# Aqasch/TensorRL-QAS

Measured on AMD Instinct MI355X. Metric: VQE env-steps/sec, higher is better.
Workload: dtype f64

## Files before the change

tensorrl-qas_amd/csrc/ham_layout.h:

```cpp
#pragma once
#include "vqe_geo.h"

#include <algorithm>
#include <cmath>
#include <cstddef>
#include <map>
#include <string>
#include <type_traits>
#include <vector>

namespace vqe {

struct HamHost {
  std::vector<uint32_t> gx_all;
  std::vector<std::vector<int>> group_terms;
  std::vector<uint64_t> hx, hz;
  std::vector<double> hcr, hci;
  bool group_has_im(int g) const {
    for (int k : group_terms[g]) if (hci[k] != 0.0) return true;
    return false;
  }
};

inline bool ham_from_paulis(int n, int n_terms, const uint64_t* xmask, const uint64_t* zmask, const double* coeff, HamHost& H) {
// ... 228 lines not shown
inline SwzChoice choose_bank_swizzle(int lt, const std::vector<uint32_t>& urec, const std::vector<uint32_t>& addr) {
  const size_t NT = (size_t)1 << lt, nu = urec.size();
  std::vector<uint8_t> lo, hi;
  size_t n_scored = 0;
  for (size_t u = 0; u < nu; ++u) {
    if (!urec[u]) continue;
    ++n_scored;
    for (size_t t = 0; t < NT; ++t) {
      const uint32_t p = addr[((u / kUnitTrip) * NT + t) * kUnitTrip + u % kUnitTrip] >> 4;
      lo.push_back((uint8_t)(p & 15u));
      hi.push_back((uint8_t)((p >> 4) & 15u));
    }
  }
  uint8_t grp[4][16];
  for (int g = 0, cnt[4] = {0, 0, 0, 0}; g < 64; ++g) {
    const int k = ((g >> 5) << 1) | (((g >> 2) ^ (g >> 3) ^ (g >> 4)) & 1);
    grp[k][cnt[k]++] = (uint8_t)g;
  }
  auto table = [](const uint32_t (&c)[4]) {
    uint64_t t = 0;
    for (uint32_t v = 0; v < 16; ++v) {
      uint32_t code = 0;
      for (int k = 0; k < 4; ++k) if ((v >> k) & 1u) code ^= c[k];
      t |= (uint64_t)code << (4 * v);
    }
    return t;
  };
  auto score = [&](uint64_t swz, double* worst) {
    size_t tot = 0;
    int w = 1;
    for (size_t i = 0; i < n_scored * NT; i += 64)
      for (int k = 0; k < 4; ++k) {
        int seen[16] = {0}, m = 0;
        for (int l = 0; l < 16; ++l) {
          const size_t j = i + grp[k][l];
          const int s = lo[j] ^ (int)((swz >> (4 * hi[j])) & 15u);
          m = std::max(m, ++seen[s]);
        }
        tot += m;
        w = std::max(w, m);
      }
    if (worst) *worst = w;
    return n_scored ? (double)tot / (double)(n_scored * NT / 16) : 1.0;
  };
  SwzChoice r{0, 1.0, 1.0, 1.0, 1.0};
  if (!n_scored || lt < 8) return r;
  r.mean0 = r.mean = score(0, &r.worst0);
  r.worst = r.worst0;
  const uint32_t starts[2][4] = {{0u, 0u, 0u, 0u}, {1u, 15u, 2u, 12u}};
  for (const auto& st : starts) {
    uint32_t c[4] = {st[0], st[1], st[2], st[3]};
    double best = score(table(c), nullptr);
    for (int sweep = 0; sweep < 4; ++sweep) {
      bool moved = false;
      for (int k = 0; k < 4; ++k)
        for (uint32_t v = 0; v < 16; ++v) {
          const uint32_t keep = c[k];
          c[k] = v;
          const double s = score(table(c), nullptr);
          if (s < best) { best = s; moved = true; } else c[k] = keep;
        }
      if (!moved) break;
    }
    if (best < r.mean) { r.mean = best; r.swz = table(c); }
  }
  if (r.swz) score(r.swz, &r.worst);
  return r;
}

struct HamLayout {
  std::vector<uint32_t> gx;
  std::vector<int32_t> tab_r, tab_i;
  std::vector<double> tables;
  int has_diag = 0;
  int n_real = 0;
  IndexMap im;
  int n_cls = 0;
  uint32_t mrow[16] = {0};
  uint64_t swz = 0;
  double mean0 = 1.0, worst0 = 1.0, mean = 1.0, worst = 1.0;
  std::vector<uint32_t> urec, uaddr;
  std::vector<double> utab;
  std::vector<int32_t> term_off{0};
  std::vector<uint32_t> term_z;
  std::vector<double> term_cr, term_ci;
};

namespace layout_detail {

constexpr const char* kTooLarge = "Hamiltonian too large for the LDS-resident path";

inline bool classify_sparse_groups(const HamHost& H, int n, int unit_F, const std::vector<int>& mine,
                                   std::vector<char>& sparse, std::vector<uint32_t>& dense_xs, std::vector<int>& hole_freq) {
  const IndexMap id = identity_map(n);
  bool any_sparse = false;
  std::vector<double> D;
  std::vector<uint32_t> act;
  std::vector<int> fixed;
  for (int g : mine) {
    const uint32_t x = H.gx_all[g];
    if (!x || H.group_has_im(g)) continue;
    const int sel = top_bit(x);
    double scale;
    pair_table(H, g, id, n, sel, D, &scale, act);
    const int patterns = choose_fixed_bits(n, sel, unit_F, act, fixed);
    const int units = patterns << (unit_F - (int)fixed.size());
    if (2 * units <= (1 << unit_F)) {
      sparse[g] = 1;
      any_sparse = true;
      for (int b : fixed) ++hole_freq[b];
      ++hole_freq[sel];
    } else {
      dense_xs.push_back(x);
    }
  }
  return any_sparse;
}

inline bool build_units(const HamHost& H, int n, int lt, const std::vector<int>& mine, const std::vector<char>& sparse,
                        HamLayout& L, std::string& err) {
  const int unit_F = n - 1 - lt;
  const size_t NT = (size_t)1 << lt;
  std::vector<double> D;
  std::vector<uint32_t> act;
  std::vector<int> fixed;
  for (int g : mine) {
    if (!sparse[g]) continue;
    const uint32_t x = L.im.map_x(H.gx_all[g]);
    const int sel = top_bit(x);
    double scale;
    pair_table(H, g, L.im, n, sel, D, &scale, act);
    choose_fixed_bits(n, sel, unit_F, act, fixed);
    for (int b = n - 1; b >= 0 && (int)fixed.size() < unit_F; --b)
      if (b != sel && std::find(fixed.begin(), fixed.end(), b) == fixed.end()) fixed.push_back(b);
    uint32_t fmask = 0;
    for (int b : fixed) fmask |= 1u << b;
    std::vector<uint32_t> keys;
    for (uint32_t p0 : act) keys.push_back(p0 & fmask);
    std::sort(keys.begin(), keys.end());
    keys.erase(std::unique(keys.begin(), keys.end()), keys.end());
    for (uint32_t s : keys) {
      L.urec.push_back(x << 4);
      for (size_t t = 0; t < NT; ++t) {
        uint32_t p0 = s, tb = 0;
        for (int b = 0; b < n; ++b)
          if (!((fmask >> b) & 1u) && b != sel) { p0 |= (uint32_t)((t >> tb) & 1u) << b; ++tb; }
        const size_t q = ((size_t)(p0 >> (sel + 1)) << sel) | (p0 & (((size_t)1 << sel) - 1));
        const double d = D[q];
        L.utab.push_back(std::fabs(d) > kUnitZeroTol * scale ? d : 0.0);
        L.uaddr.push_back(p0 << 4);
      }
    }
  }
  if (L.utab.size() * sizeof(double) + (size_t)kUnitUnroll * NT * sizeof(double) > 0x7FFFFFFFu) { err = kTooLarge; return false; }
  while (L.urec.size() % kUnitUnroll) {
    L.urec.push_back(0u);
    L.utab.resize(L.utab.size() + NT, 0.0);
    L.uaddr.resize(L.uaddr.size() + NT, 0u);
  }
  auto by_trip = [&](auto& v) {
    std::remove_reference_t<decltype(v)> t(v.size());
    const size_t n_trips = L.urec.size() / kUnitTrip;
    for (size_t T = 0; T < n_trips; ++T)
      for (size_t j = 0; j < (size_t)kUnitTrip; ++j)
        for (size_t th = 0; th < NT; ++th)
          t[(T * NT + th) * kUnitTrip + j] = v[(T * kUnitTrip + j) * NT + th];
    v.swap(t);
  };
  by_trip(L.utab);
  by_trip(L.uaddr);
  return true;
}

inline bool build_group_list(const HamHost& H, int n, bool lds_path, bool reg_path, int lt, std::vector<int> mine,
                             const std::vector<char>& sparse, HamLayout& L, std::string& err) {
  const size_t dim = (size_t)1 << n;
  const IndexMap& im = L.im;
  auto gxm = [&](int g) { return im.map_x(H.gx_all[g]); };
  auto rank_of = [&](int g) {
    if (H.group_has_im(g)) return 3;
    const uint32_t x = gxm(g);
    if (x == 0) return 0;
    return reg_path && (x >> lt) ? 1 : 2;
  };
  if (lds_path)
    std::stable_sort(mine.begin(), mine.end(), [&](int a, int b) {
      return rank_of(a) != rank_of(b) ? rank_of(a) < rank_of(b) : top_bit(gxm(a)) > top_bit(gxm(b));
    });
  auto add_dummy = [&](uint32_t xd) {
    L.gx.push_back(xd);
    L.term_off.push_back((int32_t)L.term_z.size());
    L.tab_r.push_back((int32_t)L.tables.size());
    L.tab_i.push_back(-1);
    L.tables.resize(L.tables.size() + dim / 2, 0.0);
  };
  int cur_rank = 0;
  auto enter_section = [&](int rank) {
    if (lds_path) {
      if (cur_rank <= 1 && rank >= 2) while (L.n_cls % energy_pd(n)) { add_dummy(1u << lt); ++L.n_cls; ++L.n_real; }
      if (cur_rank <= 2 && rank >= 3) while ((L.n_real - L.n_cls) % energy_pd(n)) { add_dummy(1u); ++L.n_real; }
    }
    cur_rank = rank;
  };
  std::vector<uint32_t> pidx;
  for (int g : mine) {
    if (sparse[g]) continue;
    const uint32_t x = gxm(g);
    const bool has_im = H.group_has_im(g);
    const int rank = rank_of(g);
    enter_section(rank);
    L.gx.push_back(x);
    for (int k : H.group_terms[g]) {
      L.term_z.push_back(im.map_z((uint32_t)H.hz[k]));
      L.term_cr.push_back(H.hcr[k]);
      L.term_ci.push_back(H.hci[k]);
    }
    L.term_off.push_back((int32_t)L.term_z.size());
    if (!lds_path) {
      L.tab_r.push_back(0);
      L.tab_i.push_back(has_im ? 0 : -1);
      continue;
    }
    if (rank == 0) L.has_diag = 1; else if (!has_im) ++L.n_real;
    if (rank == 1) ++L.n_cls;
    const size_t len = x == 0 ? dim : dim / 2;
    if (L.tables.size() + 2 * len > 0x7FFFFFFFu) { err = kTooLarge; return false; }
    L.tab_r.push_back((int32_t)L.tables.size());
    L.tables.resize(L.tables.size() + len, 0.0);
    if (has_im) { L.tab_i.push_back((int32_t)L.tables.size()); L.tables.resize(L.tables.size() + len, 0.0); }
    else L.tab_i.push_back(-1);
    double* tr = L.tables.data() + L.tab_r.back();
    double* ti = has_im ? L.tables.data() + L.tab_i.back() : nullptr;
    pidx.resize(len);
    for (size_t q = 0; q < len; ++q) {
      if (x == 0) pidx[q] = (uint32_t)q;
      else if (rank == 1) {
        const uint32_t t = (uint32_t)((q >> 1) & (((size_t)1 << lt) - 1));
        const uint32_t j = (uint32_t)(((q >> (lt + 1)) << 1) | (q & 1));
        pidx[q] = t | (insert0(j, top_bit(x) - lt) << lt);
      } else {
        pidx[q] = insert0((uint32_t)q, top_bit(x));
      }
    }
    for (int k : H.group_terms[g]) {
      const uint32_t z = im.map_z((uint32_t)H.hz[k]);
      const double factor = x == 0 ? 1.0 : 2.0;
      add_sign_term(tr, 1, pidx, z, factor, H.hcr[k]);
      if (ti) add_sign_term(ti, 1, pidx, z, factor, H.hci[k]);
    }
  }
  enter_section(4);
  return true;
}

}

inline bool plan_hamiltonian(const HamHost& H, int n, bool lds_path, int rank, int world, bool units_on, HamLayout& L,
                             std::string& err) {
  using namespace layout_detail;
  L = HamLayout{};
  const std::vector<int> mine = shard_groups(H, lds_path, rank, world);
  const bool reg_path = lds_path && n >= kRegMinQubits;
  const int lt = geo_lt(n);
  const int unit_F = n - 1 - lt;
  L.im = identity_map(n);
  std::vector<char> sparse(H.gx_all.size(), 0);
  bool any_sparse = false;
  if (lds_path && n >= kUnitMinQubits && units_on && unit_F >= 1) {
    std::vector<int> hole_freq(n, 0);
    std::vector<uint32_t> dense_xs;
    any_sparse = classify_sparse_groups(H, n, unit_F, mine, sparse, dense_xs, hole_freq);
    if (any_sparse && reg_path)
      L.im = choose_permutation(n, lt, dense_xs, hole_freq);
  }
  if (reg_path && !any_sparse) {
    std::vector<uint32_t> xs;
    for (int g : mine) if (H.gx_all[g] && !H.group_has_im(g)) xs.push_back(H.gx_all[g]);
    L.im = choose_index_map(n, lt, xs);
  }
  if (any_sparse && !build_units(H, n, lt, mine, sparse, L, err)) return false;
  if (!build_group_list(H, n, lds_path, reg_path, lt, mine, sparse, L, err)) return false;
  if (reg_path && !L.urec.empty() && L.gx.size() == (size_t)(L.has_diag + L.n_cls)) {
    const SwzChoice sw = choose_bank_swizzle(lt, L.urec, L.uaddr);
    L.swz = sw.swz; L.mean0 = sw.mean0; L.worst0 = sw.worst0; L.mean = sw.mean; L.worst = sw.worst;
  }
  if (L.swz) {
    for (uint32_t& a : L.uaddr) a = swz_slot(L.swz, a >> 4) << 4;
    for (uint32_t& x : L.urec) x = swz_slot(L.swz, x >> 4) << 4;
  }
  for (int i = 0; i < 16; ++i) {
    uint32_t row = L.im.row[i];
    for (int k = 0; i < 4 && k < 4; ++k)
      if ((L.swz >> (4 * (1 << k)) >> i) & 1u) row ^= L.im.row[4 + k];
    L.mrow[i] = row;
  }
  return true;
}

struct GradTables {
  std::vector<uint32_t> gx;
  std::vector<int64_t> off;
  std::vector<int32_t> cplx;
  std::vector<double> tab;
};

inline void plan_grad_tables(const HamHost& H, int n, bool lds_path, int rank, int world, GradTables& T) {
  T = GradTables{};
  const size_t dim = (size_t)1 << n;
  std::vector<uint32_t> rep;
  for (int g : shard_groups(H, lds_path, rank, world)) {
    const uint32_t x = H.gx_all[g];
    const bool im = H.group_has_im(g);
    rep.resize(x == 0 ? dim : dim / 2);
    for (size_t q = 0; q < rep.size(); ++q) rep[q] = x == 0 ? (uint32_t)q : insert0((uint32_t)q, top_bit(x));
    T.gx.push_back(x);
    T.off.push_back((int64_t)T.tab.size());
    T.cplx.push_back(im ? 1 : 0);
    const size_t base = T.tab.size();
    T.tab.resize(base + (im ? 2 : 1) * rep.size(), 0.0);
    double* t = T.tab.data() + base;
    for (int k : H.group_terms[g]) {
      add_sign_term(t, im ? 2 : 1, rep, (uint32_t)H.hz[k], 1.0, H.hcr[k]);
      if (im) add_sign_term(t + 1, 2, rep, (uint32_t)H.hz[k], 1.0, H.hci[k]);
    }
  }
}

}
```

tensorrl-qas_amd/csrc/vqe_api.hip:

```cpp
#include "../../include/vqe_hip.h"
#include "vqe_device.h"
#include "vqe_devbuf.h"
#include "vqe_stream.h"
#include "vqe_dm.h"
#include "vqe_dm_batch.h"
#include "vqe_dm_grad.h"
#include "vqe_grad.h"
#include "vqe_lbfgs.h"
#include "vqe_stream_lbfgs.h"
#include "vqe_lanczos.h"
#include "vqe_qjump.h"
#include "vqe_stream_qjump.h"
#include "ham_layout.h"
#include "dm_host.h"
#include "env_step_host.h"

#include <algorithm>
#include <cassert>
#include <cmath>
#include <cstdio>
#include <cstdlib>
#include <cstring>
#include <dlfcn.h>
#include <map>
// ... 30 lines not shown
  hipStream_t own_stream = nullptr, stream = nullptr;
  hipEvent_t ev0 = nullptr, ev1 = nullptr;
  float last_ms = 0.f;
  std::string err;

  DevBuf<double2> init;
  HamHost ham_host;
  int shard_rank = 0, shard_world = 1;
  int amp_rank = 0, amp_world = 1;
  bool ham_set = false;
  DevBuf<uint32_t> d_gx, d_term_z;
  DevBuf<double> d_term_cr, d_term_ci, d_tables;
  DevBuf<int32_t> d_tab_r, d_tab_i;

  DevBuf<int32_t> d_term_off;
  DevBuf<uint32_t> d_urec;
  DevBuf<uint32_t> d_uaddr;
  DevBuf<double> d_utab;
  HamDev ham{};
  double unit_score[4] = {1.0, 1.0, 1.0, 1.0};
  NoiseCfg noise{0.0, 0.0, 0ull, 0ull, 0.0};
  double pauli_w1[3] = {}, pauli_w2[15] = {};
  NoisePauliTab pauli_tab{};
  DevBuf<NoisePauliTab> d_pauli_tab;

  std::vector<GateRec> circ;
  int circ_params = -1;

  int batch = 0;
  int64_t total_params = 0;
  int max_ops = 0, max_params = 0, max_pair = 0;
  std::vector<int64_t> h_par_begin;
  std::vector<int32_t> h_par_count;
  DevBuf<GateRec> d_gates;
  DevBuf<int64_t> d_gate_begin, d_par_begin, d_scratch_begin;
  DevBuf<int32_t> d_gate_count, d_par_count, d_nfev, d_new_gate, d_order;
  bool has_new_gate = false;
  std::vector<int32_t> h_gate_count;
  std::vector<GateRec> h_gates;
  std::vector<int64_t> h_gate_begin;
  std::vector<double> h_theta;
  std::vector<int32_t> h_new_gate;
  DevBuf<GateRec> d_gates2;
  DevBuf<int64_t> d_gate_begin2, d_par_begin2;
  DevBuf<int32_t> d_gate_count2, d_par_count2;
  DevBuf<double> d_theta, d_x, d_xraw, d_f, d_scratch;
  DevBuf<double2> d_state;
  DevBuf<unsigned long long> d_dbg;
  DevBuf<double> d_trace;
  bool trace_on = false;
  int trace_maxfun = 0, trace_stride = 0, trace_batch = 0;
  int noise_mode = 0;
  DevBuf<double2> dm_rho;
  DevBuf<double> dm_S, dm_partial, dm_cr, dm_ci;
  DevBuf<uint32_t> dm_gx, dm_tz;
  DevBuf<int32_t> dm_toff;
  int dm_groups = 0, dm_blocks_last = 0;
  float dm_gpu_ms = 0.f;
  bool last_run_dm = false;
  hipEvent_t dm_ev0 = nullptr, dm_ev1 = nullptr;
  uint64_t dm_ham_gen = ~0ull;
  int dm_batched = 0;
  size_t dm_auto_cap = 0;
  int64_t dm_info[4] = {0, 0, 0, 0};
  DevBufExact<double2> dmb_rho;
  DevBuf<double> dmb_partial;
  DmPlanSlot dmb_full, dmb_pre;
  bool dm_grad = false;
  DmKraus kraus;
  DmKraus channels;
  bool dm_rot2 = false;
  DevBuf<double> dmg_part;
  DevBuf<int32_t> dmg_active;
  DevBuf<double> ls_xres, ls_fres;
  DevBuf<int32_t> ls_nfres, ls_running;
  DevBuf<double> d_cob_x0;
  DevBuf<int32_t> d_cob_active;
  void* comm = nullptr;
  int comm_world = 0;
  StreamWork sw;
  uint64_t gen = 0;
  uint64_t ham_ver = 0, grad_ham_ver = ~0ull;
  DevBuf<uint32_t> g_gx;
  DevBuf<int64_t> g_off;
  DevBuf<int32_t> g_cplx;
  DevBuf<double> g_tab, d_grad;
  DevBuf<double2> g_lam;
  GradHam gham{};
  DevBuf<double> lb_work;
  DevBuf<int32_t> lb_nit, lb_status;
  int lb_batch = 0;
  bool stream_grad = false, stream_states_undone = false;
  bool stream_lbfgs = false;
  DevBufExact<StreamLbfgsRec> lb_rec;
  int kraus_traj = 0;
  uint64_t qj_ver = 0, qj_tab_ver = ~0ull;
  DevBuf<double> qj_K1, qj_W1, qj_K2, qj_W2, qj_e;
  DevBuf<int32_t> qj_jumps;
  DevBuf<long long> qj_jsum;
  int qj_n1 = 0, qj_n2 = 0;
  int64_t qj_info[4] = {0, 0, 0, 0};
  int qj_traj_batch = 0;
  int qj_jsum_batch = 0;
  int sq_resident = 0;
  size_t sq_auto_cap = 0;
  int64_t sq_info[4] = {0, 0, 0, 0};
  DevBuf<QjOp> sq_ops;
  DevBuf<uint32_t> sq_masks;
  DevBuf<int32_t> sq_meta, sq_jpos;
  DevBuf<double2> sq_cs;
  DevBuf<double> sq_part, sq_kmat;
  LzWork lz;
};

#ifdef VQE_STAMPS
static unsigned long long cby_out_[8];
#endif
namespace {

int fail(vqe_t* h, int code, const std::string& msg) {
  if (h) h->err = msg; else g_create_error = msg;
  return code;
}

template <class T>
int upload(vqe_t* h, DevBuf<T>& b, const T* src, size_t n) {
  HIP_TRY(h, b.reserve(n ? n : 1));
  if (n) HIP_TRY(h, hipMemcpyAsync(b.p, src, n * sizeof(T), hipMemcpyHostToDevice, h->stream));
  return VQE_OK;
}
template <class T>
int upload(vqe_t* h, DevBuf<T>& b, const std::vector<T>& src) { return upload(h, b, src.data(), src.size()); }

int build_hamiltonian(vqe_t* h, HamHost* H, int rank, int world) {
  static const bool units_on = [] { const char* e = std::getenv("VQE_UNITS"); return !(e && e[0] == '0'); }();
  HamLayout L;
  std::string err;
  if (!plan_hamiltonian(H ? *H : h->ham_host, h->n, h->lds_path, rank, world, units_on, L, err))
    return fail(h, VQE_EINVAL, err);
  if (H) h->ham_host = std::move(*H);
  h->shard_rank = rank;
  h->shard_world = world;
  h->ham_set = true;
  ++h->gen;
  ++h->ham_ver;
  VQE_TRY(upload(h, h->d_gx, L.gx));
  VQE_TRY(upload(h, h->d_tab_r, L.tab_r));
  VQE_TRY(upload(h, h->d_tab_i, L.tab_i));
  VQE_TRY(upload(h, h->d_tables, L.tables));
  VQE_TRY(upload(h, h->d_term_off, L.term_off));
  VQE_TRY(upload(h, h->d_term_z, L.term_z));
  VQE_TRY(upload(h, h->d_term_cr, L.term_cr));
  VQE_TRY(upload(h, h->d_term_ci, L.term_ci));
  VQE_TRY(upload(h, h->d_urec, L.urec));
  VQE_TRY(upload(h, h->d_uaddr, L.uaddr));
  VQE_TRY(upload(h, h->d_utab, L.utab));
  HIP_TRY(h, hipStreamSynchronize(h->stream));
  HamDev& d = h->ham;
  d.n_groups = (int)L.gx.size();
  d.n_terms = (int)L.term_z.size();
  d.n_units = (int)L.urec.size();
  d.gx = h->d_gx.p; d.tab_r = h->d_tab_r.p; d.tab_i = h->d_tab_i.p; d.tables = h->d_tables.p;
  d.urec = h->d_urec.p; d.uaddr = h->d_uaddr.p; d.utab = h->d_utab.p;
  d.term_off = h->d_term_off.p; d.term_z = h->d_term_z.p; d.term_cr = h->d_term_cr.p; d.term_ci = h->d_term_ci.p;
  d.has_diag = L.has_diag; d.n_real = L.n_real; d.n_cls = L.n_cls;
  std::copy(L.mrow, L.mrow + 16, d.mrow);
  d.swz = L.swz;
  h->unit_score[0] = L.mean0; h->unit_score[1] = L.worst0; h->unit_score[2] = L.mean; h->unit_score[3] = L.worst;
  return VQE_OK;
}

int check_gates(vqe_t* h, int64_t n_gates, const int32_t* kind, const int32_t* q0,
                const int32_t* q1, const int32_t* pidx, int n_params) {
  for (int64_t i = 0; i < n_gates; ++i) {
    const int k = kind[i];
    if (k < 0 || k > VQE_GATE_RZZ) return fail(h, VQE_EINVAL, "unknown gate kind");
    if (q0[i] < 0 || q0[i] >= h->n) return fail(h, VQE_EINVAL, "gate qubit out of range");
    if (k == VQE_GATE_CNOT || k == VQE_GATE_DEPOL2 || gate_is_rot2(k)) {
      if (q1[i] < 0 || q1[i] >= h->n || q1[i] == q0[i])
        return fail(h, VQE_EINVAL, "two-qubit gate needs two distinct qubits in range");
    }
    if (gate_is_rot(k)) {
      if (pidx[i] < 0 || pidx[i] >= n_params)
        return fail(h, VQE_EINVAL, "rotation parameter index out of range");
    }
  }
  return VQE_OK;
}

enum class Run { Energy, Minimize, State, EnvStep, Reduce };

void set_env_step(const vqe_t* h, BatchArgs& A) {
  A.env_step = 1;
  A.new_gate = h->has_new_gate ? h->d_new_gate.p : nullptr;
}

#ifdef VQE_ONLY_N
using LdsSizes = std::integer_sequence<int, VQE_ONLY_N>;
#else
using LdsSizes = std::integer_sequence<int, 1, 2, 3, 4, 5, 6, 7, 8, 9, 10, 11, 12, 13>;
#endif
template <class F, int... Ns>
int dispatch_n(vqe_t* h, const char* refusal, F f, std::integer_sequence<int, Ns...>) {
  int rc = 0;
  const bool found = (... || (h->n == Ns && ((rc = f(std::integral_constant<int, Ns>{})), true)));
  return found ? rc : fail(h, VQE_EINVAL, refusal);
}

constexpr int kWideMinN = 6;
bool wide_launch(int n, int max_params) {
  static const bool wide_on = [] { const char* e = std::getenv("VQE_WIDE_UPDATE"); return !(e && e[0] == '0'); }();
  return n >= kWideMinN && wide_on && max_params > 64;
}

const char* lds_launch_refusal(int n, size_t lds, int max_ops, size_t lds_per_cu) {
  if (lds > lds_per_cu) return "circuit too large for the LDS-resident path (gates + parameters)";
  if (n >= kRegMinQubits && (size_t)max_ops > ((size_t)1 << n))
    return "circuit too large for the LDS-resident path (more than 2^n rotations)";
  return nullptr;
}

void report_placement(int n, int max_ops, int max_pair, int max_params, int n_groups, int nvar, bool wide, size_t lds_per_cu,
                      int64_t out[8]) {
  const bool resident = cobyla_resident_bytes(n, max_ops, max_params, n_groups, max_pair) != 0;
  const CobPlacement p = cobyla_placement(n, wide, resident, nvar);
  const size_t lds = lds_bytes(n, max_ops, max_params, n_groups, max_pair, wide);
  out[0] = p.resident ? VQE_COBYLA_RESIDENT : p.staged ? VQE_COBYLA_STAGED : p.block ? VQE_COBYLA_BLOCK
           : p.rows ? VQE_COBYLA_ROWS : VQE_COBYLA_GLOBAL;
  out[1] = p.pad;
  out[2] = p.words;
  out[3] = (int64_t)lds;
  out[4] = p.split;
  out[5] = (int64_t)cobyla_tile_bytes(n, max_params, wide);
  out[6] = (int64_t)cobyla_resident_bytes(n, max_ops, max_params, n_groups, max_pair);
  out[7] = lds_launch_refusal(n, lds, max_ops, lds_per_cu) == nullptr;
}

template <int N>
int launch_lds(vqe_t* h, Run mode, BatchArgs A) {
  if (mode == Run::EnvStep) set_env_step(h, A);
  const bool minimize = mode == Run::Minimize || mode == Run::EnvStep;
  constexpr bool kHasWide = N >= kWideMinN;
  const bool wide = minimize && wide_launch(N, A.max_params);
  size_t lds = lds_bytes(N, A.max_ops, A.max_params, A.ham.n_groups, A.max_pair, wide);
  static const long lds_pad = [] { const char* e = std::getenv("VQE_LDS_PAD"); return e ? std::atol(e) : 0L; }();
  if (lds_pad > 0) lds += (size_t)lds_pad;
  if (const char* why = lds_launch_refusal(N, lds, A.max_ops, (size_t)h->lds_per_cu)) return fail(h, VQE_EINVAL, why);
  const bool noisy = A.noise.p1 > 0.0 || A.noise.p2 > 0.0;
  constexpr bool kW = false;
  void (*const kernel)(BatchArgs) =
      mode == Run::Energy ? k_lds_energy<N>
      : !minimize ? k_lds_state<N>
      : wide ? (noisy ? k_lds_minimize<N, kHasWide, true> : k_lds_minimize<N, kHasWide, false>)
             : (noisy ? k_lds_minimize<N, kW, true> : k_lds_minimize<N, kW, false>);
  const void* fn = (const void*)kernel;
  HIP_TRY(h, hipFuncSetAttribute(fn, hipFuncAttributeMaxDynamicSharedMemorySize, (int)lds));
  {
    hipFuncAttributes fa;
    HIP_TRY(h, hipFuncGetAttributes(&fa, fn));
    if (fa.sharedSizeBytes != 0) return fail(h, VQE_ESTATE, "LDS-resident kernel was built with static LDS");
  }
  h->last_wg_per_cu = std::max(1, std::min(8, (int)(h->lds_per_cu / lds)));
  HIP_TRY(h, hipEventRecord(h->ev0, h->stream));
  const dim3 grid(mode == Run::State ? 1 : A.batch), block(Geo<N>::NT);
  hipLaunchKernelGGL(kernel, grid, block, lds, h->stream, A);
  HIP_TRY(h, hipGetLastError());
  HIP_TRY(h, hipEventRecord(h->ev1, h->stream));
  return VQE_OK;
}

int dispatch_lds(vqe_t* h, Run mode, const BatchArgs& A) {
  return dispatch_n(h, "n_qubits outside the LDS-resident range",
                    [&](auto n) -> int { return launch_lds<decltype(n)::value>(h, mode, A); }, LdsSizes{});
}

NoiseCfg launch_noise(const vqe_t* h) {
  NoiseCfg nz = h->noise;
  if (h->pauli_tab.has1) nz.p1 = h->pauli_tab.cum1[2];
  if (h->pauli_tab.has2) nz.p2 = h->pauli_tab.cum2[14];
  nz.pauli = (h->pauli_tab.has1 || h->pauli_tab.has2) ? h->d_pauli_tab.p : nullptr;
  return nz;
}
bool pauli_noise_on(const vqe_t* h) {
  const NoiseCfg nz = launch_noise(h);
  return nz.p1 > 0.0 || nz.p2 > 0.0;
}
void set_channels(vqe_t* h) {
  h->channels = h->kraus;
  if (h->kraus.n1 == 0 && h->pauli_tab.has1) { pauli_kraus(h->pauli_w1, 2, h->channels.K1); h->channels.n1 = 4; }
  if (h->kraus.n2 == 0 && h->pauli_tab.has2) { pauli_kraus(h->pauli_w2, 4, h->channels.K2); h->channels.n2 = 16; }
}

BatchArgs make_args(vqe_t* h) {
  BatchArgs A{};
  A.n = h->n;
  A.batch = h->batch;
  A.gates = h->d_gates.p;
  A.gate_begin = h->d_gate_begin.p;
  A.gate_count = h->d_gate_count.p;
  A.par_begin = h->d_par_begin.p;
  A.par_count = h->d_par_count.p;
  A.order = h->d_order.p;
  A.theta = h->d_theta.p;
  A.xout = h->d_x.p;
  A.xraw = h->d_xraw.p;
  A.new_gate = nullptr;
  A.env_step = 0;
  A.fout = h->d_f.p;
  A.nfev = h->d_nfev.p;
  A.scratch = h->d_scratch.p;
  A.scratch_begin = h->d_scratch_begin.p;
  A.init = h->init.p;
  A.ham = h->ham;
  A.noise = launch_noise(h);
// ... 2121 lines not shown
```

tensorrl-qas_amd/csrc/vqe_device.h:

```cpp
#pragma once
#include <hip/hip_runtime.h>
#include <stdint.h>
#ifdef VQE_STAMPS
__device__ unsigned long long g_cby_dbg[8];
__device__ unsigned long long g_cby_in_out[2];
__device__ long long g_cby_t0_unused;
#if defined(__HIP_DEVICE_COMPILE__)
#define CBY_STAMP_RESET() long long cby_t0_ = (long long)__builtin_readcyclecounter(); (void)cby_t0_
#define CBY_STAMP(k)                                                                               \
  {                                                                                                \
    const long long t_ = (long long)__builtin_readcyclecounter();                                  \
    if (ctx.tid == 0 && Ctx::nth > 1) __hip_atomic_fetch_add(&g_cby_dbg[k], (unsigned long long)(t_ - cby_t0_), __ATOMIC_RELAXED, __HIP_MEMORY_SCOPE_AGENT); \
    cby_t0_ = (long long)__builtin_readcyclecounter();                                             \
  }
#else
#define CBY_STAMP_RESET()
#define CBY_STAMP(k)
#endif
#endif
#include "cobyla_m0.h"
#include "vqe_geo.h"
#include "noise_pauli.h"

namespace vqe {
// ... 873 lines not shown
      const double* treal = tables + __builtin_amdgcn_readfirstlane(L.gm[g0].off_r);
      VQE_E_CTX(VQE_E_XFETCH(g0))
      xq = VQE_E_XFETCH(g0 + 1);
      VQE_E_LOAD(0, aA, bA)
      for (int g = g0; g < g1; g += PD) {
#pragma unroll
        for (int j = 0; j < PD; ++j) {
          {
            const int sl = (j + PD - 1) % PD;
            int gr = (j == 0) ? (g == g0 ? g0 + PD - 1 : g - 1 + PD) : g + j - 1 + PD;
            gr = gr < g1 ? gr : g1 - 1;
            const double* t = treal + (size_t)(gr - g0) * (DIM / 2);
#pragma unroll
            for (int k = 0; k < NP; ++k) buf[sl][k] = t[tid + (uint32_t)k * kThreads];
          }
          VQE_E_LOAD(1, aB, bB)
          __builtin_amdgcn_sched_barrier(0);
          VQE_E_COMP(0, aA, bA, buf[j])
          __builtin_amdgcn_sched_barrier(0);
          VQE_E_CTX(xq)
          xq = VQE_E_XFETCH(g + j + 2);
          VQE_E_LOAD(0, aA, bA)
          __builtin_amdgcn_sched_barrier(0);
          VQE_E_COMP(1, aB, bB, buf[j])
          __builtin_amdgcn_sched_barrier(0);
        }
      }
#undef VQE_E_CTX
#undef VQE_E_XFETCH
#undef VQE_E_LOAD
#undef VQE_E_COMP
    } else {
      for (int g = g0; g < g1; g += PD) {
        const int gn = g + PD < g1 ? g + PD : g;
#pragma unroll
        for (int j = 0; j < PD; ++j) {
          VQE_ENERGY_CONSUME(g + j, buf[j])
          const double* t = tables + __builtin_amdgcn_readfirstlane(L.gm[gn + j].off_r);
#pragma unroll
          for (int k = 0; k < NP; ++k) {
            const uint32_t q = tid + (uint32_t)k * kThreads;
            buf[j][k] = (FULL || q < DIM / 2) ? t[q] : 0.0;
          }
          __builtin_amdgcn_sched_barrier(0);
        }
      }
    }
  }
}

template <int N>
__device__ __forceinline__ void energy_imag_lds(const Lds& L, const double* __restrict__ tables, int g1, int g2,
                                                double& acc0) {
  constexpr int kThreads = Geo<N>::NT;
  constexpr uint32_t DIM = 1u << N;
  constexpr int NP = (DIM / 2 + kThreads - 1) / kThreads;
  constexpr bool FULL = DIM / 2 >= kThreads;
  const uint32_t tid = threadIdx.x;
  for (int g = g1; g < g2; ++g) {
    const GroupMeta m = L.gm[g];
    const double* tr = tables + m.off_r;
    const double* ti = tables + m.off_i;
    double part = 0.0;
#pragma unroll
    for (int k = 0; k < NP; ++k) {
      const uint32_t q = tid + (uint32_t)k * kThreads;
      if (FULL || q < DIM / 2) {
        const uint32_t p0 = insert0(q, m.hb);
        const double2 b = L.psi[p0], a = L.psi[p0 ^ m.x];
        part += (a.x * b.x + a.y * b.y) * tr[q] - (a.x * b.y - a.y * b.x) * ti[q];
      }
    }
    acc0 += part;
  }
}

template <int N>
__device__ __forceinline__ void unit_energy(const Lds& L, const HamDev& H, double& acc0, double& acc1);

template <int N>
__device__ __forceinline__ double lds_energy(const Lds& L, const HamDev& H) {
  constexpr int kThreads = Geo<N>::NT;
  constexpr uint32_t DIM = 1u << N;
  constexpr int NA = (DIM + kThreads - 1) / kThreads;
  const uint32_t tid = threadIdx.x;
  const double* __restrict__ tables = H.tables;
  double acc0 = 0.0, acc1 = 0.0;
  int g0 = 0;
  if (H.has_diag) {
    const double* t = tables + L.gm[0].off_r;
#pragma unroll
    for (int k = 0; k < NA; ++k) {
      const uint32_t p = tid + (uint32_t)k * kThreads;
      if (DIM >= kThreads || p < DIM) {
        const double2 a = L.psi[p];
        const double v = (a.x * a.x + a.y * a.y) * t[p];
        if (k & 1) acc1 += v; else acc0 += v;
      }
    }
    g0 = 1;
  }
  const int g1 = g0 + H.n_real;
  energy_real_lds<N>(L, tables, g0, g1, acc0, acc1);
  energy_imag_lds<N>(L, tables, g1, H.n_groups, acc0);
  if constexpr (N >= kUnitMinQubits && N - 1 - Geo<N>::LT >= 1) unit_energy<N>(L, H, acc0, acc1);
  return block_sum<Geo<N>::NW>(acc0 + acc1, L.red);
}


__device__ __forceinline__ __amdgpu_buffer_rsrc_t table_rsrc(const void* p) {
  return __builtin_amdgcn_make_buffer_rsrc((void*)p, 0, -1, 0x00020000);
}
__device__ __forceinline__ double2 buf_load_d2(__amdgpu_buffer_rsrc_t rs, uint32_t voff, uint32_t soff) {
  const v4i_t v = __builtin_amdgcn_raw_buffer_load_b128(rs, (int)voff, (int)soff, 0);
  return make_double2(__hiloint2double(v.y, v.x), __hiloint2double(v.w, v.z));
}
__device__ __forceinline__ double buf_load_d(__amdgpu_buffer_rsrc_t rs, uint32_t voff, uint32_t soff) {
  const v2i_t v = __builtin_amdgcn_raw_buffer_load_b64(rs, (int)voff, (int)soff, 0);
  return __hiloint2double(v.y, v.x);
}
__device__ __forceinline__ double2 lds_load_d2(lds_cbyte* base, uint32_t off) {
  const d2v_t v = *(const __attribute__((address_space(3))) d2v_t*)(base + off);
  return make_double2(v.x, v.y);
}

__device__ __forceinline__ void pair_fma4(double& acc0, double& acc1, const double2& a0, const double2& a1,
                                          const double2& a2, const double2& a3, const double2 (&b)[4], double d0,
                                          double d1, double d2, double d3) {
  double t0, t1, t2, t3;
  asm("v_mul_f64 %2, %6, %14\n\tv_mul_f64 %3, %8, %16\n\tv_mul_f64 %4, %10, %18\n\tv_mul_f64 %5, %12, %20\n\t"
      "v_fmac_f64 %2, %7, %15\n\tv_fmac_f64 %3, %9, %17\n\tv_fmac_f64 %4, %11, %19\n\tv_fmac_f64 %5, %13, %21\n\t"
      "v_fmac_f64 %0, %2, %22\n\tv_fmac_f64 %1, %3, %23\n\tv_fmac_f64 %0, %4, %24\n\tv_fmac_f64 %1, %5, %25"
      : "+v"(acc0), "+v"(acc1), "=&v"(t0), "=&v"(t1), "=&v"(t2), "=&v"(t3)
      : "v"(a0.x), "v"(a0.y), "v"(a1.x), "v"(a1.y), "v"(a2.x), "v"(a2.y), "v"(a3.x), "v"(a3.y),
        "v"(b[0].x), "v"(b[0].y), "v"(b[1].x), "v"(b[1].y), "v"(b[2].x), "v"(b[2].y), "v"(b[3].x), "v"(b[3].y),
        "v"(d0), "v"(d1), "v"(d2), "v"(d3));
}
__device__ __forceinline__ void pair_fma2(double& acc0, double& acc1, const double2& a0, const double2& a1,
                                          const double2 (&b)[2], double d0, double d1) {
  double t0, t1;
  asm("v_mul_f64 %2, %4, %8\n\tv_mul_f64 %3, %6, %10\n\t"
      "v_fmac_f64 %2, %5, %9\n\tv_fmac_f64 %3, %7, %11\n\t"
      "v_fmac_f64 %0, %2, %12\n\tv_fmac_f64 %1, %3, %13"
      : "+v"(acc0), "+v"(acc1), "=&v"(t0), "=&v"(t1)
      : "v"(a0.x), "v"(a0.y), "v"(a1.x), "v"(a1.y), "v"(b[0].x), "v"(b[0].y), "v"(b[1].x), "v"(b[1].y),
        "v"(d0), "v"(d1));
}
__device__ __forceinline__ void pair_fma1(double& acc0, const double2& a0, const double2 (&b)[1], double d0) {
  double t0;
  asm("v_mul_f64 %1, %2, %4\n\tv_fmac_f64 %1, %3, %5\n\tv_fmac_f64 %0, %1, %6"
      : "+v"(acc0), "=&v"(t0) : "v"(a0.x), "v"(a0.y), "v"(b[0].x), "v"(b[0].y), "v"(d0));
}

__device__ __forceinline__ double2 lds_load_abs(uint32_t addr) {
  const d2v_t v = *(const __attribute__((address_space(3))) d2v_t*)(uintptr_t)addr;
  return make_double2(v.x, v.y);
}
typedef uint32_t u32x4_t __attribute__((ext_vector_type(4)));
typedef __attribute__((address_space(4))) const u32x4_t const_u32x4;

template <int N>
__device__ __forceinline__ void unit_energy(const Lds& L, const HamDev& H, double& acc0, double& acc1) {
  constexpr int LT = Geo<N>::LT;
  constexpr int U = kUnitTrip;
  static_assert(kUnitUnroll == 3 * kUnitTrip, "three trips per turn of the loop (ring of three table buffers)");
  static_assert(U == 4, "a trip is [thread][unit of the trip]: two 16-byte table loads and one 16-byte address load per thread");
  constexpr uint32_t TRIP_BYTES = (uint32_t)(8 * U) << LT;
  constexpr uint32_t TRIP_ABYTES = (uint32_t)(4 * U) << LT;
  const int nu = __builtin_amdgcn_readfirstlane(H.n_units);
  if (nu <= 0) return;
  uint32_t tid = threadIdx.x;
  asm volatile("" : "+v"(tid));
  const __amdgpu_buffer_rsrc_t ru = table_rsrc(H.utab);
  const __amdgpu_buffer_rsrc_t ra = table_rsrc(H.uaddr);
  const const_u32x4* rec = (const const_u32x4*)H.urec;
  double d[3][U];
  u32x4_t ad[3];
  u32x4_t X = rec[0];
  const uint32_t tid32 = tid << 5;
  const uint32_t tid16 = tid << 4;
  auto load_trip = [&](double (&dst)[U], u32x4_t& adst, uint32_t first_unit) {
    const uint32_t trip = first_unit / U;
    const v4i_t av = __builtin_amdgcn_raw_buffer_load_b128(ra, (int)tid16, (int)(trip * TRIP_ABYTES), 0);
    adst = u32x4_t{(uint32_t)av.x, (uint32_t)av.y, (uint32_t)av.z, (uint32_t)av.w};
    const uint32_t soff = trip * TRIP_BYTES;
    const double2 lo = buf_load_d2(ru, tid32, soff), hi = buf_load_d2(ru, tid32 + 16u, soff);
    dst[0] = lo.x; dst[1] = lo.y; dst[2] = hi.x; dst[3] = hi.y;
  };
  load_trip(d[0], ad[0], 0u);
  load_trip(d[1], ad[1], (uint32_t)(U < nu ? U : 0));
  const int last = nu - U;
  for (int u = 0; u < nu; u += 3 * U) {
#pragma unroll
    for (int k = 0; k < 3; ++k) {
      const int ub = u + k * U;
      const int u1 = ub + U < last ? ub + U : last;
      const int u2 = ub + 2 * U < last ? ub + 2 * U : last;
      double2 pa[U], pb[U];
      uint32_t a[U], ax[U];
#pragma unroll
      for (int j = 0; j < U; ++j) {
        a[j] = ad[k][j];
        asm("v_xor_b32 %0, %1, %2" : "=v"(ax[j]) : "s"(X[j]), "v"(a[j]));
      }
      __builtin_amdgcn_sched_barrier(0);
#pragma unroll
      for (int j = 0; j < U; ++j) {
        pb[j] = lds_load_abs(a[j]);
        pa[j] = lds_load_abs(ax[j]);
      }
      load_trip(d[(k + 2) % 3], ad[(k + 2) % 3], (uint32_t)u2);
      __builtin_amdgcn_sched_barrier(0);
      X = rec[u1 / U];
      __builtin_amdgcn_sched_barrier(0);
#pragma unroll
      for (int j = 0; j < U; ++j) {
        const double v = (pa[j].x * pb[j].x + pa[j].y * pb[j].y) * d[k][j];
        if (j & 1) acc1 += v; else acc0 += v;
      }
      __builtin_amdgcn_sched_barrier(0);
    }
  }
}

struct NoHook { __device__ __forceinline__ void operator()() const {} };

template <int N, class Hook = NoHook>
__device__ __forceinline__ double reg_energy(const Lds& L, const HamDev& H, Hook after_pairs = Hook()) {
  constexpr int kThreads = Geo<N>::NT;
  constexpr uint32_t DIM = 1u << N;
  constexpr int LT = Geo<N>::LT;
  constexpr int R = N - LT;
  constexpr int NA = 1 << R;
  constexpr int NP = NA / 2;
  constexpr int HP = NP / 2;
  constexpr int PD = energy_pd(N);
  static_assert(NP >= 2 && NP <= 8 && PD % 2 == 0, "register energy path: 2..8 pairs per thread");
  uint32_t tid = threadIdx.x;
  asm volatile("" : "+v"(tid));
  const uint32_t stid = swz_slot(H.swz, tid);
  const double* __restrict__ tables = H.tables;
  lds_cbyte* psi_l = (lds_cbyte*)L.psi;
  double2 own[NA];
#pragma unroll
  for (int r = 0; r < NA; ++r) own[r] = lds_load_d2(psi_l, (stid + (uint32_t)r * kThreads) << 4);
  double acc0 = 0.0, acc1 = 0.0;
  int g0 = 0;
  if (H.has_diag) {
    const __amdgpu_buffer_rsrc_t rd = table_rsrc(tables + __builtin_amdgcn_readfirstlane(L.gm[0].off_r));
#pragma unroll
    for (int r = 0; r < NA; ++r) {
      const double v = (own[r].x * own[r].x + own[r].y * own[r].y) * buf_load_d(rd, (tid + (uint32_t)r * kThreads) << 3, 0);
      if (r & 1) acc1 += v; else acc0 += v;
    }
    g0 = 1;
  }
  const int gc = g0 + H.n_cls;
  if (g0 < gc) {
    const int ncls = H.n_cls;
    constexpr uint32_t GSTRIDE = DIM * 4;
    double2 buf[PD][NP / 2];
    const __amdgpu_buffer_rsrc_t rt = table_rsrc(tables + __builtin_amdgcn_readfirstlane(L.gm[g0].off_r));
    uint32_t voff[NP / 2];
#pragma unroll
    for (int k = 0; k < NP / 2; ++k) voff[k] = (tid + (uint32_t)k * kThreads) << 4;
#pragma unroll
    for (int j = 0; j < PD - 1; ++j) {
#pragma unroll
      for (int k = 0; k < NP / 2; ++k) buf[j][k] = buf_load_d2(rt, voff[k], (uint32_t)j * GSTRIDE);
      __builtin_amdgcn_sched_barrier(0);
    }
#pragma unroll
    for (int k = 0; k < NP / 2; ++k) buf[PD - 1][k] = make_double2(0.0, 0.0);
    double2 bA[HP], bB[HP];
    uint2 mh[2];
    uint4 mo[2][2];
    const uint32_t tid16 = stid << 4;
    uint32_t tb;
    int ccls;
#define VQE_R_FETCH(S, GI)                                                                         \
    {                                                                                              \
      const ClsMeta* cm_ = L.cm + ((GI) < ncls ? (GI) : ncls - 1);                                 \
      mh[S] = *(const uint2*)cm_;                                                                  \
      mo[S][0] = *(const uint4*)cm_->off;                                                          \
      if constexpr (NP > 4) mo[S][1] = *(const uint4*)(cm_->off + 4);                             \
    }
#define VQE_R_OFF(S, J) ((J) == 0 ? mo[S][0].x : (J) == 1 ? mo[S][0].y : (J) == 2 ? mo[S][0].z : (J) == 3 ? mo[S][0].w : \
                         (J) == 4 ? mo[S][1].x : (J) == 5 ? mo[S][1].y : (J) == 6 ? mo[S][1].z : mo[S][1].w)
#define VQE_R_LOAD(S, HH, PB)                                                                      \
    _Pragma("unroll") for (int kk = 0; kk < HP; ++kk)                                             \
      PB[kk] = lds_load_d2(psi_l, tb + VQE_R_OFF(S, (HH) * HP + kk));
#define VQE_R_OWN(C, J) own[(((J) >> (C)) << ((C) + 1)) | ((J) & ((1 << (C)) - 1))]
#define VQE_R_DV(D, J) (((J) & 1) ? D[(J) / 2].y : D[(J) / 2].x)
#define VQE_R_COMP_C(C, HH, PB, D)                                                                 \
    if constexpr (HP == 4)                                                                         \
      pair_fma4(acc0, acc1, VQE_R_OWN(C, (HH) * 4), VQE_R_OWN(C, (HH) * 4 + 1), VQE_R_OWN(C, (HH) * 4 + 2),     \
                VQE_R_OWN(C, (HH) * 4 + 3), PB, VQE_R_DV(D, (HH) * 4), VQE_R_DV(D, (HH) * 4 + 1),            \
                VQE_R_DV(D, (HH) * 4 + 2), VQE_R_DV(D, (HH) * 4 + 3));                                       \
    else if constexpr (HP == 2)                                                                    \
      pair_fma2(acc0, acc1, VQE_R_OWN(C, (HH) * 2), VQE_R_OWN(C, (HH) * 2 + 1), PB, VQE_R_DV(D, (HH) * 2),     \
                VQE_R_DV(D, (HH) * 2 + 1));                                                                  \
    else                                                                                           \
      pair_fma1(acc0, VQE_R_OWN(C, (HH)), PB, VQE_R_DV(D, (HH)));
#define VQE_R_BODY(C, JJ)                                                                          \
    {                                                                                              \
      VQE_R_COMP_C(C, 0, bA, buf[JJ])                                                              \
      __builtin_amdgcn_sched_barrier(0);                                                           \
      tb = tid16 ^ mh[((JJ) + 1) & 1].x;                                                           \
      VQE_R_LOAD(((JJ) + 1) & 1, 0, bA)                                                            \
      __builtin_amdgcn_sched_barrier(0);                                                           \
      VQE_R_COMP_C(C, 1, bB, buf[JJ])                                                              \
    }
    VQE_R_FETCH(0, 0)
    VQE_R_FETCH(1, 1)
    tb = tid16 ^ mh[0].x;
    VQE_R_LOAD(0, 0, bA)
    for (int g = 0; g < ncls; g += PD) {
#pragma unroll
      for (int j = 0; j < PD; ++j) {
        {
          const int sl = (j + PD - 1) % PD;
          int gr = (j == 0) ? (g == 0 ? PD - 1 : g - 1 + PD) : g + j - 1 + PD;
          gr = gr < ncls ? gr : ncls - 1;
          const uint32_t soff = (uint32_t)gr * GSTRIDE;
#pragma unroll
          for (int k = 0; k < NP / 2; ++k) buf[sl][k] = buf_load_d2(rt, voff[k], soff);
        }
        ccls = __builtin_amdgcn_readfirstlane((int)mh[j & 1].y);
        VQE_R_LOAD(j & 1, 1, bB)
        VQE_R_FETCH(j & 1, g + j + 2)
        __builtin_amdgcn_sched_barrier(0);
        switch (ccls) {
          case 0: VQE_R_BODY(0, j) break;
          case 1: VQE_R_BODY(1, j) break;
          case 2: if constexpr (R > 2) VQE_R_BODY(2, j) break;
          default: if constexpr (R > 3) VQE_R_BODY(3, j) break;
        }
        __builtin_amdgcn_sched_barrier(0);
      }
    }
#undef VQE_R_FETCH
#undef VQE_R_OFF
#undef VQE_R_LOAD
#undef VQE_R_OWN
#undef VQE_R_DV
#undef VQE_R_COMP_C
#undef VQE_R_BODY
  }
  after_pairs();
  unit_energy<N>(L, H, acc0, acc1);
  const int g1 = g0 + H.n_real;
  energy_real_lds<N>(L, tables, gc, g1, acc0, acc1);
  energy_imag_lds<N>(L, tables, g1, H.n_groups, acc0);
  return block_sum<Geo<N>::NW>(acc0 + acc1, L.red);
}

template <int N, bool SLOTS = false, class Hook = NoHook>
__device__ __forceinline__ double lds_evaluate(const BatchArgs& A, const Lds& L, const double* theta, int P,
                                               int p_hole = -1, Hook after_pairs = Hook(), bool cs_ready = false) {
#ifdef VQE_STAMPS
  const long long t0 = clock64();
#endif
  if constexpr (N >= kRegMinQubits) {
    run_ops_reg<N, SLOTS>(L, A.init, theta, P, p_hole, A.dbg, cs_ready);
  } else {
    load_init<N>(L, A.init);
    __syncthreads();
    run_ops<N, SLOTS>(L, theta, P, p_hole);
  }
#ifdef VQE_STAMPS
  const long long t1 = clock64();
#endif
  double e;
  if constexpr (N >= kRegMinQubits) e = reg_energy<N>(L, A.ham, after_pairs); else e = lds_energy<N>(L, A.ham);
#ifdef VQE_STAMPS
// ... 394 lines not shown
```

tensorrl-qas_amd/csrc/vqe_geo.h:

```cpp
#pragma once
#include <stdint.h>

#if defined(__HIPCC__)
#define VQE_HD __host__ __device__
#else
#define VQE_HD
#endif

namespace vqe {

constexpr int kThreads = 256;

#ifndef VQE_WIDE_MIN
#define VQE_WIDE_MIN 13
#endif
constexpr int kWideMinQubits = VQE_WIDE_MIN;

#ifndef VQE_ONE_WAVE_MAX
#define VQE_ONE_WAVE_MAX 9
#endif
constexpr int kOneWaveMaxQubits = VQE_ONE_WAVE_MAX;

#ifndef VQE_ONE_WAVE_REG
#define VQE_ONE_WAVE_REG 0
#endif
VQE_HD constexpr bool geo_one_wave(int n) { return n <= kOneWaveMaxQubits || (VQE_ONE_WAVE_REG && n == 10); }
VQE_HD constexpr int geo_lt(int n) { return n >= kWideMinQubits ? 9 : (geo_one_wave(n) ? 6 : 8); }

#ifndef VQE_WPS_SMALL
#define VQE_WPS_SMALL 2
#endif
#ifndef VQE_WPS10
#define VQE_WPS10 4
#endif
#ifndef VQE_WPS11
#define VQE_WPS11 3
#endif
template <int N>
struct Geo {
  static constexpr int NT = 1 << geo_lt(N);
  static constexpr int LT = geo_lt(N);
  static constexpr int NW = NT / 64;
  static constexpr int WPS = N == 11 ? VQE_WPS11 : (N == 10 ? (VQE_ONE_WAVE_REG ? 2 : VQE_WPS10) : (N <= 9 ? VQE_WPS_SMALL : 2));
};

constexpr int kRegMinQubits = 10;

enum : int { G_CNOT = 0, G_RX = 1, G_RY = 2, G_RZ = 3, G_DEPOL1 = 4, G_DEPOL2 = 5, G_RXX = 6, G_RYY = 7, G_RZZ = 8 };
VQE_HD constexpr bool gate_is_rot2(int k) { return k >= G_RXX && k <= G_RZZ; }
VQE_HD constexpr bool gate_is_rot(int k) { return (k >= G_RX && k <= G_RZ) || gate_is_rot2(k); }
struct GateRec { int32_t kind, q0, q1, pidx; };

struct PreAction { int skip, skip_end, hole; };
VQE_HD inline PreAction pre_action(const GateRec* g, int G, int new_gate) {
  if (new_gate < 0) return PreAction{-1, 0, -1};
  const GateRec r = g[new_gate];
  PreAction pa{new_gate, new_gate + 1, gate_is_rot(r.kind) ? r.pidx : -1};
  if (new_gate + 1 < G) {
    const GateRec fo = g[new_gate + 1];
    if ((fo.kind == G_DEPOL1 && r.kind >= G_RX && r.kind <= G_RZ && fo.q0 == r.q0) ||
        (fo.kind == G_DEPOL2 && r.kind == G_CNOT && fo.q0 == r.q0 && fo.q1 == r.q1))
      pa.skip_end = new_gate + 2;
  }
  return pa;
}

VQE_HD constexpr int energy_pd(int n) { return n >= 11 ? 2 : 4; }

VQE_HD inline uint32_t swz_slot(uint64_t swz, uint32_t p) {
  return p ^ (uint32_t)((swz >> (((p >> 4) & 15u) << 2)) & 15u);
}
constexpr int kUnitMinQubits = 8;
constexpr int kUnitTrip = 4;
constexpr int kUnitUnroll = 3 * kUnitTrip;
constexpr double kUnitZeroTol = 0x1p-44;

}
```

Measured before the change: 13320.

## Pad unit arrays for prefetch and stage LDS waits per unit in energy loop

The unit-energy loop now prefetches two trips ahead into host-padded arrays (kUnitAhead zero entries), so it no longer needs clamped min() indices and instead advances scalar byte offsets. LDS reads are issued as raw ds_read_b128 with explicit staged lgkmcnt waits, and each unit's multiply-accumulate is written as inline asm. The goal is to overlap LDS latency with FMA work per unit and to drop index arithmetic. In exchange it relies on hand-counted waitcnt values matching the number of outstanding LDS reads, and it uses slightly more device memory for the padding.

```diff
diff --git a/tensorrl-qas_amd/csrc/ham_layout.h b/tensorrl-qas_amd/csrc/ham_layout.h
--- a/tensorrl-qas_amd/csrc/ham_layout.h
+++ b/tensorrl-qas_amd/csrc/ham_layout.h
@@ -404,7 +404,7 @@
       }
     }
   }
-  if (L.utab.size() * sizeof(double) + (size_t)kUnitUnroll * NT * sizeof(double) > 0x7FFFFFFFu) { err = kTooLarge; return false; }
+  if (L.utab.size() * sizeof(double) + (size_t)(kUnitUnroll + kUnitAhead) * NT * sizeof(double) > 0x7FFFFFFFu) { err = kTooLarge; return false; }
   while (L.urec.size() % kUnitUnroll) {
     L.urec.push_back(0u);
     L.utab.resize(L.utab.size() + NT, 0.0);
@@ -549,6 +549,22 @@
   return true;
 }
 
+struct UnitArrays {
+  int n_units = 0;
+  std::vector<uint32_t> urec, uaddr;
+  std::vector<double> utab;
+};
+inline UnitArrays unit_arrays(const HamLayout& L, int lt) {
+  UnitArrays A;
+  A.n_units = (int)L.urec.size();
+  if (!A.n_units) return A;
+  const size_t NT = (size_t)1 << lt, total = L.urec.size() + (size_t)kUnitAhead;
+  A.urec = L.urec;   A.urec.resize(total, 0u);
+  A.uaddr = L.uaddr; A.uaddr.resize(total * NT, 0u);
+  A.utab = L.utab;   A.utab.resize(total * NT, 0.0);
+  return A;
+}
+
 struct GradTables {
   std::vector<uint32_t> gx;
   std::vector<int64_t> off;
diff --git a/tensorrl-qas_amd/csrc/vqe_api.hip b/tensorrl-qas_amd/csrc/vqe_api.hip
--- a/tensorrl-qas_amd/csrc/vqe_api.hip
+++ b/tensorrl-qas_amd/csrc/vqe_api.hip
@@ -206,14 +206,15 @@
   VQE_TRY(upload(h, h->d_term_z, L.term_z));
   VQE_TRY(upload(h, h->d_term_cr, L.term_cr));
   VQE_TRY(upload(h, h->d_term_ci, L.term_ci));
-  VQE_TRY(upload(h, h->d_urec, L.urec));
-  VQE_TRY(upload(h, h->d_uaddr, L.uaddr));
-  VQE_TRY(upload(h, h->d_utab, L.utab));
+  const UnitArrays UA = unit_arrays(L, geo_lt(h->n));
+  VQE_TRY(upload(h, h->d_urec, UA.urec));
+  VQE_TRY(upload(h, h->d_uaddr, UA.uaddr));
+  VQE_TRY(upload(h, h->d_utab, UA.utab));
   HIP_TRY(h, hipStreamSynchronize(h->stream));
   HamDev& d = h->ham;
   d.n_groups = (int)L.gx.size();
   d.n_terms = (int)L.term_z.size();
-  d.n_units = (int)L.urec.size();
+  d.n_units = UA.n_units;
   d.gx = h->d_gx.p; d.tab_r = h->d_tab_r.p; d.tab_i = h->d_tab_i.p; d.tables = h->d_tables.p;
   d.urec = h->d_urec.p; d.uaddr = h->d_uaddr.p; d.utab = h->d_utab.p;
   d.term_off = h->d_term_off.p; d.term_z = h->d_term_z.p; d.term_cr = h->d_term_cr.p; d.term_ci = h->d_term_ci.p;
diff --git a/tensorrl-qas_amd/csrc/vqe_device.h b/tensorrl-qas_amd/csrc/vqe_device.h
--- a/tensorrl-qas_amd/csrc/vqe_device.h
+++ b/tensorrl-qas_amd/csrc/vqe_device.h
@@ -1049,12 +1049,21 @@
       : "+v"(acc0), "=&v"(t0) : "v"(a0.x), "v"(a0.y), "v"(b[0].x), "v"(b[0].y), "v"(d0));
 }
 
-__device__ __forceinline__ double2 lds_load_abs(uint32_t addr) {
-  const d2v_t v = *(const __attribute__((address_space(3))) d2v_t*)(uintptr_t)addr;
-  return make_double2(v.x, v.y);
-}
 typedef uint32_t u32x4_t __attribute__((ext_vector_type(4)));
 typedef __attribute__((address_space(4))) const u32x4_t const_u32x4;
+
+__device__ __forceinline__ void unit_lds_read(d2v_t& dst, uint32_t addr) {
+  asm volatile("ds_read_b128 %0, %1" : "=v"(dst) : "v"(addr) : "memory");
+}
+template <int CNT>
+__device__ __forceinline__ void unit_wait(d2v_t& p0, d2v_t& p1) {
+  asm volatile("s_waitcnt lgkmcnt(%2)" : "+v"(p0), "+v"(p1) : "n"(CNT));
+}
+__device__ __forceinline__ void unit_fma(double& acc, const d2v_t& a, const d2v_t& b, double d) {
+  double t;
+  asm("v_mul_f64 %1, %3, %5\n\tv_fmac_f64 %1, %2, %4\n\tv_fmac_f64 %0, %1, %6"
+      : "+v"(acc), "=&v"(t) : "v"(a.x), "v"(a.y), "v"(b.x), "v"(b.y), "v"(d));
+}
 
 template <int N>
 __device__ __forceinline__ void unit_energy(const Lds& L, const HamDev& H, double& acc0, double& acc1) {
@@ -1070,30 +1079,28 @@
   asm volatile("" : "+v"(tid));
   const __amdgpu_buffer_rsrc_t ru = table_rsrc(H.utab);
   const __amdgpu_buffer_rsrc_t ra = table_rsrc(H.uaddr);
-  const const_u32x4* rec = (const const_u32x4*)H.urec;
+  typedef __attribute__((address_space(4))) const unsigned char const_byte;
+  const_byte* rec = (const_byte*)H.urec;
+  static_assert(kUnitAhead == 2 * kUnitTrip, "the loop prefetches two trips beyond the one it accumulates");
   double d[3][U];
   u32x4_t ad[3];
-  u32x4_t X = rec[0];
+  u32x4_t X = *(const const_u32x4*)rec;
   const uint32_t tid32 = tid << 5;
   const uint32_t tid16 = tid << 4;
-  auto load_trip = [&](double (&dst)[U], u32x4_t& adst, uint32_t first_unit) {
-    const uint32_t trip = first_unit / U;
-    const v4i_t av = __builtin_amdgcn_raw_buffer_load_b128(ra, (int)tid16, (int)(trip * TRIP_ABYTES), 0);
+  auto load_trip = [&](double (&dst)[U], u32x4_t& adst, uint32_t soff_a, uint32_t soff_t) {
+    const v4i_t av = __builtin_amdgcn_raw_buffer_load_b128(ra, (int)tid16, (int)soff_a, 0);
     adst = u32x4_t{(uint32_t)av.x, (uint32_t)av.y, (uint32_t)av.z, (uint32_t)av.w};
-    const uint32_t soff = trip * TRIP_BYTES;
-    const double2 lo = buf_load_d2(ru, tid32, soff), hi = buf_load_d2(ru, tid32 + 16u, soff);
+    const double2 lo = buf_load_d2(ru, tid32, soff_t), hi = buf_load_d2(ru, tid32 + 16u, soff_t);
     dst[0] = lo.x; dst[1] = lo.y; dst[2] = hi.x; dst[3] = hi.y;
   };
-  load_trip(d[0], ad[0], 0u);
-  load_trip(d[1], ad[1], (uint32_t)(U < nu ? U : 0));
-  const int last = nu - U;
-  for (int u = 0; u < nu; u += 3 * U) {
+  load_trip(d[0], ad[0], 0u, 0u);
+  load_trip(d[1], ad[1], TRIP_ABYTES, TRIP_BYTES);
+  uint32_t st = 2u * TRIP_BYTES, sa = 2u * TRIP_ABYTES, sr = 16u;
+  const uint32_t st_end = ((uint32_t)nu / U + 2u) * TRIP_BYTES;
+  do {
 #pragma unroll
     for (int k = 0; k < 3; ++k) {
-      const int ub = u + k * U;
-      const int u1 = ub + U < last ? ub + U : last;
-      const int u2 = ub + 2 * U < last ? ub + 2 * U : last;
-      double2 pa[U], pb[U];
+      d2v_t pa[U], pb[U];
       uint32_t a[U], ax[U];
 #pragma unroll
       for (int j = 0; j < U; ++j) {
@@ -1103,21 +1110,28 @@
       __builtin_amdgcn_sched_barrier(0);
 #pragma unroll
       for (int j = 0; j < U; ++j) {
-        pb[j] = lds_load_abs(a[j]);
-        pa[j] = lds_load_abs(ax[j]);
-      }
-      load_trip(d[(k + 2) % 3], ad[(k + 2) % 3], (uint32_t)u2);
+        unit_lds_read(pb[j], a[j]);
+        unit_lds_read(pa[j], ax[j]);
+      }
+      load_trip(d[(k + 2) % 3], ad[(k + 2) % 3], sa, st);
       __builtin_amdgcn_sched_barrier(0);
-      X = rec[u1 / U];
+      X = *(const const_u32x4*)(rec + sr);
+      st += TRIP_BYTES; sa += TRIP_ABYTES; sr += 16u;
       __builtin_amdgcn_sched_barrier(0);
-#pragma unroll
-      for (int j = 0; j < U; ++j) {
-        const double v = (pa[j].x * pb[j].x + pa[j].y * pb[j].y) * d[k][j];
-        if (j & 1) acc1 += v; else acc0 += v;
-      }
+      unit_wait<6>(pb[0], pa[0]);
+      unit_fma(acc0, pa[0], pb[0], d[k][0]);
       __builtin_amdgcn_sched_barrier(0);
-    }
-  }
+      unit_wait<4>(pb[1], pa[1]);
+      unit_fma(acc1, pa[1], pb[1], d[k][1]);
+      __builtin_amdgcn_sched_barrier(0);
+      unit_wait<2>(pb[2], pa[2]);
+      unit_fma(acc0, pa[2], pb[2], d[k][2]);
+      __builtin_amdgcn_sched_barrier(0);
+      unit_wait<0>(pb[3], pa[3]);
+      unit_fma(acc1, pa[3], pb[3], d[k][3]);
+      __builtin_amdgcn_sched_barrier(0);
+    }
+  } while (st < st_end);
 }
 
 struct NoHook { __device__ __forceinline__ void operator()() const {} };
diff --git a/tensorrl-qas_amd/csrc/vqe_geo.h b/tensorrl-qas_amd/csrc/vqe_geo.h
--- a/tensorrl-qas_amd/csrc/vqe_geo.h
+++ b/tensorrl-qas_amd/csrc/vqe_geo.h
@@ -73,6 +73,7 @@
 constexpr int kUnitMinQubits = 8;
 constexpr int kUnitTrip = 4;
 constexpr int kUnitUnroll = 3 * kUnitTrip;
+constexpr int kUnitAhead = 2 * kUnitTrip;
 constexpr double kUnitZeroTol = 0x1p-44;
 
 }
```

Result: faster. 13670, median of 6 (+2.6%).
